# haotiansun14/rl-rep

Measured on NVIDIA B200. Metric: agent updates/sec, higher is better.
Workload: dtype tf32

## Files before the change

### rlrep_b200/csrc/gemm_chain.cu

```cuda
#include <algorithm>
#include <cmath>
#include <cstdlib>
#include <cstring>

#include "common.cuh"
#include "gemm_chain.cuh"
#include "ptx.cuh"

namespace rlrep {

namespace {

constexpr int kThreads = 320;
constexpr int kEpiWarps = 8;
constexpr int kStages = 6;
constexpr int kCW = 16;
constexpr int kTwPitch = kCW + 4;
constexpr int kMaxBn = 128;
constexpr int kBM = 128, kBK = 32;
constexpr int kABytes = kBM * kBK * 4;
constexpr int kStageBytes = kABytes + kMaxBn * kBK * 4;
constexpr int kTbufFloats = kEpiWarps * 32 * kTwPitch;
constexpr int kSub = 4, kCtrStride = 32;
constexpr int kDbgItems = 16, kDbgEvents = 10;
constexpr int kSmemBytes = kStages * kStageBytes + 1024 + 256 + kTbufFloats * 4;
static_assert(kSmemBytes <= 227 * 1024, "chain kernel shared memory");

__device__ __forceinline__ void red_release_add(unsigned* p, unsigned v) {
  asm volatile("red.release.gpu.global.add.u32 [%0], %1;" ::"l"(p), "r"(v) : "memory");
}
__device__ __forceinline__ unsigned atom_add_acq_rel(unsigned* p, unsigned v) {
  unsigned old;
  asm volatile("atom.acq_rel.gpu.global.add.u32 %0, [%1], %2;" : "=r"(old) : "l"(p), "r"(v) : "memory");
  return old;
}
__device__ __forceinline__ void fence_proxy_async_global() { asm volatile("fence.proxy.async.global;" ::: "memory"); }
__device__ __forceinline__ void fence_tensormap_acquire(const CUtensorMap* m) {
  asm volatile("fence.proxy.tensormap::generic.acquire.gpu [%0], 128;" ::"l"(reinterpret_cast<uint64_t>(m)) : "memory");
}
__device__ __forceinline__ unsigned ld_relaxed(const unsigned* p) {
  unsigned v;
  asm volatile("ld.relaxed.gpu.global.u32 %0, [%1];" : "=r"(v) : "l"(p) : "memory");
  return v;
}
__device__ __forceinline__ void wait_counter(const unsigned* done, int dep, int dep_tiles) {
  const unsigned* p = done + (size_t)dep * kSub * kCtrStride;
  unsigned target[kSub];
#pragma unroll
  for (int sub = 0; sub < kSub; ++sub) target[sub] = (unsigned)((dep_tiles - sub + kSub - 1) / kSub);
  long long t0 = 0;
  while (true) {
    unsigned v[kSub];
#pragma unroll
    for (int sub = 0; sub < kSub; ++sub) v[sub] = ld_relaxed(p + sub * kCtrStride);
    bool ok = true;
#pragma unroll
    for (int sub = 0; sub < kSub; ++sub) ok = ok && v[sub] >= target[sub];
    if (ok) return;
    __nanosleep(20);
    if (t0 == 0) t0 = clock64();
    if (clock64() - t0 > 4000000000LL) {
      printf("rlrep: chain dependency wait timed out (block %d, gemm %d, tiles %d, counters %u %u %u %u)\n", blockIdx.x, dep,
             dep_tiles, v[0], v[1], v[2], v[3]);
      __trap();
    }
  }
}
__device__ __forceinline__ void fence_acquire_gpu() { asm volatile("fence.acq_rel.gpu;" ::: "memory"); }

__device__ __forceinline__ void epilogue_bar() { asm volatile("bar.sync 1, 256;" ::: "memory"); }

__device__ __forceinline__ float elu_fast(float x) {
  const float n = fminf(x, 0.f);
  float p = 1.f / 5040.f;
  p = fmaf(p, n, 1.f / 720.f);
  p = fmaf(p, n, 1.f / 120.f);
  p = fmaf(p, n, 1.f / 24.f);
  p = fmaf(p, n, 1.f / 6.f);
  p = fmaf(p, n, 0.5f);
  p = fmaf(p, n, 1.f);
// ... 62 lines not shown
      if constexpr (ACT != ACT_NONE) {
#pragma unroll
        for (int e = 0; e < 4; ++e) v[e] = ACT == ACT_ELU ? elu_fast(v[e]) : apply_act(v[e], ACT < 0 ? epi.act : ACT);
      }
      if constexpr (DACT != DACT_NONE) {
        const int dact = DACT < 0 ? epi.dact : DACT;
        if (dact != DACT_NONE) {
          const float4 x = o.aux[r4];
          v[0] *= apply_dact(x.x, dact); v[1] *= apply_dact(x.y, dact); v[2] *= apply_dact(x.z, dact); v[3] *= apply_dact(x.w, dact);
        }
      }
      float4* cp = reinterpret_cast<float4*>(C + (size_t)om * ldc + on);
      if (epi.accumulate) {
        const float4 c0 = __ldcg(cp);
        v[0] += c0.x; v[1] += c0.y; v[2] += c0.z; v[3] += c0.w;
      }
      *cp = make_float4(v[0], v[1], v[2], v[3]);
    }
  }
}

__global__ void __launch_bounds__(kThreads, 1)
gemm_chain_kernel(const ChainGemmDesc* __restrict__ gemms, const ChainTask* __restrict__ tasks,
                  const int* __restrict__ task_begin, unsigned* __restrict__ done, unsigned* __restrict__ exit_ctr,
                  int n_gemms, unsigned long long* __restrict__ dbg) {
  auto stamp = [&](int item, int ev) {
    if (dbg != nullptr && item < kDbgItems) {
      unsigned long long t;
      asm volatile("mov.u64 %0, %%globaltimer;" : "=l"(t)::"memory");
      dbg[((size_t)blockIdx.x * kDbgItems + item) * kDbgEvents + ev] = t;
    }
  };
  if (threadIdx.x == 0) stamp(kDbgItems - 1, 2);
  extern __shared__ uint8_t smem_raw[];
  uint8_t* smem = reinterpret_cast<uint8_t*>((reinterpret_cast<uintptr_t>(smem_raw) + 1023) & ~uintptr_t(1023));
  uint64_t* full_bar = reinterpret_cast<uint64_t*>(smem + kStages * kStageBytes);
  uint64_t* empty_bar = full_bar + 8;
  uint64_t* acc_full = empty_bar + 8;
  uint64_t* acc_empty = acc_full + 2;
  uint32_t* tmem_slot = reinterpret_cast<uint32_t*>(acc_empty + 2);
  volatile unsigned* arrival = reinterpret_cast<volatile unsigned*>(tmem_slot + 1);
  float* tbuf = reinterpret_cast<float*>(smem + kStages * kStageBytes + 256);

  const int warp = threadIdx.x >> 5, lane = threadIdx.x & 31;
  const int t_begin = task_begin[blockIdx.x], t_end = task_begin[blockIdx.x + 1];

  if (threadIdx.x == 0) {
    for (int s = 0; s < kStages; ++s) {
      ptx::mbar_init(&full_bar[s], 1);
      ptx::mbar_init(&empty_bar[s], 1);
    }
    for (int a = 0; a < 2; ++a) {
      ptx::mbar_init(&acc_full[a], 1);
      ptx::mbar_init(&acc_empty[a], kEpiWarps);
    }
    ptx::fence_mbar_init();
  }
  if (warp == 1) {
    ptx::tmem_alloc(tmem_slot, 2 * kMaxBn);
    ptx::tmem_relinquish();
  }
  ptx::tc_fence_before_sync();
  __syncthreads();
  ptx::tc_fence_after_sync();
  const uint32_t tmem_base = *tmem_slot;

  if (warp == 0) {
    if (lane == 0) {
      int it = 0, last_gemm = -1;
      for (int t = t_begin; t < t_end; ++t) {
        const ChainTask tk = tasks[t];
        const ChainGemmDesc* g = gemms + tk.gemm;
        const int n_deps = g->n_deps;
        const int bn = g->bn, a_mn = g->a_mn, b_mn = g->b_mn;
        const int m0 = (tk.tile % g->tiles_m) * kBM, n0 = (tk.tile / g->tiles_m) * bn;
        const int kb0 = tk.split * g->kb_per_split, kb1 = min(g->nkb, kb0 + g->kb_per_split);
        int dep_id[kChainMaxDeps], dep_tiles[kChainMaxDeps];
#pragma unroll
        for (int d = 0; d < kChainMaxDeps; ++d) {
          dep_id[d] = d < n_deps ? g->dep[d] : 0;
          dep_tiles[d] = d < n_deps ? (int)g->dep_target[d] : 0;
        }
        if (tk.gemm != last_gemm) {
          fence_tensormap_acquire(&g->tmA);
          fence_tensormap_acquire(&g->tmB);
          last_gemm = tk.gemm;
        }
        stamp(t - t_begin, 0);
        if (dbg != nullptr && t - t_begin < kDbgItems)
          dbg[((size_t)blockIdx.x * kDbgItems + (t - t_begin)) * kDbgEvents + 8] =
              (unsigned long long)tk.gemm | ((unsigned long long)tk.tile << 16) | ((unsigned long long)tk.split << 40);
#pragma unroll
        for (int d = 0; d < kChainMaxDeps; ++d)
          if (d < n_deps) wait_counter(done, dep_id[d], dep_tiles[d]);
        if (n_deps > 0) {
          fence_acquire_gpu();
          fence_proxy_async_global();
        }
        stamp(t - t_begin, 1);
        const uint32_t tx = kABytes + bn * kBK * 4;
        for (int kb = kb0; kb < kb1; ++kb, ++it) {
          const int s = it % kStages;
          ptx::mbar_wait(&empty_bar[s], ((it / kStages) & 1) ^ 1);
          ptx::mbar_arrive_expect_tx(&full_bar[s], tx);
          uint8_t* a_dst = smem + s * kStageBytes;
          uint8_t* b_dst = a_dst + kABytes;
          const int k0 = kb * kBK;
          if (!a_mn) ptx::tma_load_2d(a_dst, &g->tmA, &full_bar[s], k0, m0);
          else ptx::tma_load_3d(a_dst, &g->tmA, &full_bar[s], 0, k0, m0 / 32);
          if (!b_mn) ptx::tma_load_2d(b_dst, &g->tmB, &full_bar[s], k0, n0);
          else ptx::tma_load_3d(b_dst, &g->tmB, &full_bar[s], 0, k0, n0 / 32);
        }
        stamp(t - t_begin, 2);
      }
    }
  } else if (warp == 1) {
    if (ptx::elect_one()) {
      int it = 0, tc = 0;
      for (int t = t_begin; t < t_end; ++t, ++tc) {
        const ChainTask tk = tasks[t];
        const ChainGemmDesc* g = gemms + tk.gemm;
        const int bn = g->bn, a_mn = g->a_mn, b_mn = g->b_mn;
        const int kb0 = tk.split * g->kb_per_split, kb1 = min(g->nkb, kb0 + g->kb_per_split);
        const uint32_t idesc = ptx::make_idesc_tf32(kBM, bn, a_mn != 0, b_mn != 0);
        const int acc = tc & 1;
        ptx::mbar_wait(&acc_empty[acc], ((tc >> 1) & 1) ^ 1);
        ptx::tc_fence_after_sync();
        const uint32_t d_tmem = tmem_base + acc * kMaxBn;
        for (int kb = kb0; kb < kb1; ++kb, ++it) {
          const int s = it % kStages;
          ptx::mbar_wait(&full_bar[s], (it / kStages) & 1);
          if (kb == kb0) stamp(t - t_begin, 3);
          ptx::tc_fence_after_sync();
          const uint32_t a_addr = ptx::smem_u32(smem + s * kStageBytes);
          const uint32_t b_addr = a_addr + kABytes;
#pragma unroll
          for (int k = 0; k < kBK / 8; ++k) {
            const uint64_t adesc = a_mn ? ptx::make_smem_desc(a_addr + k * 1024, 4096, 512, 1)
                                        : ptx::make_smem_desc(a_addr + k * 32, 16, 1024, 2);
            const uint64_t bdesc = b_mn ? ptx::make_smem_desc(b_addr + k * 1024, 4096, 512, 1)
                                        : ptx::make_smem_desc(b_addr + k * 32, 16, 1024, 2);
            ptx::mma_tf32_ss(d_tmem, adesc, bdesc, idesc, (kb > kb0 || k > 0) ? 1u : 0u);
          }
          ptx::mma_commit(&empty_bar[s]);
        }
        ptx::mma_commit(&acc_full[acc]);
        stamp(t - t_begin, 4);
      }
    }
  } else {
    const int q = warp & 3, half = (warp - 2) >> 2;
    float* tw = tbuf + (warp - 2) * (32 * kTwPitch);
    int tc = 0;
    for (int t = t_begin; t < t_end; ++t, ++tc) {
      const ChainTask tk = tasks[t];
      const ChainGemmDesc* g = gemms + tk.gemm;
      const Epilogue epi = g->epi;
      const int bn = g->bn, M = g->M, N = g->N, ldc = g->ldc, split_k = g->split_k;
      float* __restrict__ C = g->C;
      float* __restrict__ ws = g->ws;
      unsigned* __restrict__ tile_ctr = g->tile_ctr;
      const int m0 = (tk.tile % g->tiles_m) * kBM, n0 = (tk.tile / g->tiles_m) * bn;
      const int chunks = bn / kCW;
      const int acc = tc & 1;
      const uint32_t t_acc = tmem_base + (static_cast<uint32_t>(32 * q) << 16) + acc * kMaxBn;
      const int row = 32 * q + lane;
      ptx::mbar_wait(&acc_full[acc], (tc >> 1) & 1);
      if (threadIdx.x == 64) stamp(t - t_begin, 5);
      ptx::tc_fence_after_sync();

      bool final = true;
      const size_t part_floats = (size_t)kBM * bn;
      float* ws_tile = split_k > 1 ? ws + (size_t)tk.tile * split_k * part_floats : nullptr;
      const bool dist = split_k > 1 && g->dist != 0;
      int c_first = half, c_step = 2;
      if (split_k > 1) {
        float* part = ws_tile + (size_t)tk.split * part_floats;
#pragma unroll 1
        for (int c = half; c < chunks; c += 2) {
          if (dist && c % split_k == tk.split) continue;
          uint32_t v[kCW];
          ptx::tmem_ld_32x32b_x16(t_acc + c * kCW, v);
          ptx::tmem_ld_wait();
#pragma unroll
          for (int j = 0; j < kCW / 4; ++j)
            __stcg(reinterpret_cast<float4*>(part + ((size_t)(c * (kCW / 4) + j) * kBM + row) * 4),
                   make_float4(__uint_as_float(v[4 * j]), __uint_as_float(v[4 * j + 1]), __uint_as_float(v[4 * j + 2]),
                               __uint_as_float(v[4 * j + 3])));
        }
        epilogue_bar();
        if (threadIdx.x == 64) {
          unsigned* ctr = tile_ctr + tk.tile;
          const unsigned old = atom_add_acq_rel(ctr, 1u);
          if (dist) {
            if (old + 1 < (unsigned)split_k) {
              unsigned long long t0 = 0;
              unsigned spins = 0;
              while (ld_relaxed(ctr) < (unsigned)split_k) {
                __nanosleep(20);
                if ((++spins & 0xfff) == 0) {
                  unsigned long long now;
                  asm volatile("mov.u64 %0, %%globaltimer;" : "=l"(now));
                  if (t0 == 0) t0 = now;
                  else if (now - t0 > 2000000000ull) __trap();
                }
              }
              fence_acquire_gpu();
            }
          } else if (old == (unsigned)(split_k - 1)) {
            *ctr = 0;
          }
          *arrival = old;
          stamp(t - t_begin, 6);
        }
        epilogue_bar();
        final = dist || *arrival == (unsigned)(split_k - 1);
        if (dist) {
          c_first = tk.split + split_k * half;
          c_step = 2 * split_k;
        }
      }
      if (final) {
        const bool use_aux = epi.dact != DACT_NONE;
        const bool vec_ok = (ldc & 3) == 0 && aligned16(C) && (N & 3) == 0 &&
                            (!use_aux || ((epi.ld_aux & 3) == 0 && aligned16(epi.aux))) &&
                            (!epi.pre_out || ((epi.ld_pre & 3) == 0 && aligned16(epi.pre_out))) &&
                            (!epi.bias || aligned16(epi.bias)) && (!epi.r1_v || aligned16(epi.r1_v));
#pragma unroll 1
        for (int c = c_first; c < chunks; c += c_step) {
          const int gn0 = n0 + c * kCW;
          const bool fast = vec_ok && gn0 + kCW <= N;
          ChunkOperands ops;
          if (fast) chunk_prefetch(ops, epi, M, m0 + 32 * q, gn0, lane);
          float a[kCW];
          if (split_k == 1) {
            uint32_t v[kCW];
            ptx::tmem_ld_32x32b_x16(t_acc + c * kCW, v);
            ptx::tmem_ld_wait();
#pragma unroll
            for (int e = 0; e < kCW; ++e) a[e] = __uint_as_float(v[e]);
          } else {
            const float* base = ws_tile + ((size_t)(c * (kCW / 4)) * kBM + row) * 4;
            float4 nxt[kCW / 4];
            const int s_first = tk.split == 0 ? 1 : 0;
#pragma unroll
            for (int j = 0; j < kCW / 4; ++j)
              nxt[j] = __ldcg(reinterpret_cast<const float4*>(base + (size_t)s_first * part_floats + (size_t)j * kBM * 4));
#pragma unroll 1
            for (int s = 0; s < split_k; ++s) {
              if (s == tk.split) {
                uint32_t v[kCW];
                ptx::tmem_ld_32x32b_x16(t_acc + c * kCW, v);
                ptx::tmem_ld_wait();
                if (s == 0) {
#pragma unroll
                  for (int e = 0; e < kCW; ++e) a[e] = __uint_as_float(v[e]);
                } else {
#pragma unroll
                  for (int e = 0; e < kCW; ++e) a[e] += __uint_as_float(v[e]);
                }
                continue;
              }
              float4 cur[kCW / 4];
// ... 21 lines not shown
          __syncwarp();
          if (fast) {
#define RLREP_CSTORE(A, D) chain_store_rows<A, D>(epi, ops, tw, C, ldc, M, m0 + 32 * q, gn0, lane)
            RLREP_EPILOGUE_SWITCH(epi, RLREP_CSTORE);
#undef RLREP_CSTORE
          } else if (gn0 < N) {
            const int piece = lane & 3, rsub = lane >> 2;
#pragma unroll 1
            for (int r4 = 0; r4 < 4; ++r4) {
              const int r = r4 * 8 + rsub, om = m0 + 32 * q + r;
              if (om >= M) continue;
#pragma unroll 1
              for (int e = 0; e < 4; ++e) {
                const int on = gn0 + 4 * piece + e;
                if (on < N) {
                  float* cp = C + (size_t)om * ldc + on;
                  *cp = chain_epilogue_scalar(epi, tw[r * kTwPitch + 4 * piece + e], om, on, cp);
                }
              }
            }
          }
          __syncwarp();
        }
        if (threadIdx.x == 64) stamp(t - t_begin, 9);
        epilogue_bar();
        if (threadIdx.x == 64) {
          fence_proxy_async_global();
          const int pub = dist ? tk.tile * split_k + tk.split : tk.tile;
          red_release_add(done + ((size_t)tk.gemm * kSub + (pub % kSub)) * kCtrStride, 1u);
          stamp(t - t_begin, 7);
          if (dist) {
            unsigned* ctr = tile_ctr + tk.tile;
            if (atomicAdd(ctr, 1u) == (unsigned)(2 * split_k - 1)) *ctr = 0;
          }
        }
      }
      ptx::tc_fence_before_sync();
      __syncwarp();
      if (lane == 0) ptx::mbar_arrive(&acc_empty[acc]);
    }
  }
  ptx::tc_fence_before_sync();
  __syncthreads();
  if (warp == 1) ptx::tmem_dealloc(tmem_base, 2 * kMaxBn);
  if (threadIdx.x == 0) {
    const unsigned old = atom_add_acq_rel(exit_ctr, 1u);
    if (old == gridDim.x - 1) {
      for (int i = 0; i < n_gemms * kSub; ++i) done[(size_t)i * kCtrStride] = 0;
      *exit_ctr = 0;
      __threadfence();
    }
    stamp(kDbgItems - 1, 3);
  }
}

struct Range {
  uintptr_t lo = 0, hi = 0;
  bool overlaps(const Range& o) const { return lo < o.hi && o.lo < hi && lo != hi && o.lo != o.hi; }
};
Range range_of(const float* p, long long rows, long long ld, long long cols) {
  Range r;
  if (p == nullptr || rows <= 0 || cols <= 0) return r;
  r.lo = reinterpret_cast<uintptr_t>(p);
  r.hi = r.lo + (size_t)((rows - 1) * ld + cols) * sizeof(float);
  return r;
}
struct Footprint {
  std::vector<Range> reads, writes;
};
Footprint footprint(const GemmArgs& a) {
  Footprint f;
  f.reads.push_back(a.a_mn ? range_of(a.A, a.K, a.lda, a.M) : range_of(a.A, a.M, a.lda, a.K));
  f.reads.push_back(a.b_mn ? range_of(a.B, a.K, a.ldb, a.N) : range_of(a.B, a.N, a.ldb, a.K));
  f.reads.push_back(range_of(a.epi.bias, 1, 0, a.N));
// ... 5 lines not shown
  f.writes.push_back(range_of(a.epi.pre_out, a.M, a.epi.ld_pre, a.N));
  return f;
}
bool conflicts(const Footprint& earlier, const Footprint& later) {
  for (const Range& w : earlier.writes) {
    for (const Range& r : later.reads)
      if (w.overlaps(r)) return true;
    for (const Range& r : later.writes)
      if (w.overlaps(r)) return true;
  }
  for (const Range& w : later.writes)
    for (const Range& r : earlier.reads)
      if (w.overlaps(r)) return true;
  return false;
}

unsigned long long* g_chain_dbg = nullptr;

int env_int(const char* name, int dflt) {
  const char* e = std::getenv(name);
  return e ? std::atoi(e) : dflt;
}

bool dist_possible(int bn, int split) { return split > 1 && (bn / kCW) % split == 0; }
double plan_cost(int tiles, int nkb, int bn, int split, int share, bool dist) {
  const int kb_per = ceil_div(nkb, split);
  const double kb_bytes = kABytes + bn * kBK * 4;
  const double waves = std::ceil((double)tiles * split / share);
  const double stream = waves * kb_per * kb_bytes / 150e3;
  const double chip = (double)tiles * split * kb_per * kb_bytes / 12e6;
  if (dist) {
    return 1.5 + std::max(stream, chip) + waves * (0.25 * ceil_div(bn, 64) + 1.0 + 1.0 * ceil_div(bn / split, 64)) +
           0.1 * (split - 1);
  }
  double t = 1.5 + std::max(stream, chip) + waves * 1.0 * ceil_div(bn, 64);
  if (split > 1) t += 1.5 + 0.3 * (split - 1) * ceil_div(bn, 64);
  return t;
}

}

void set_chain_debug_buffer(unsigned long long* dev) { g_chain_dbg = dev; }

bool chain_eligible(const GemmArgs& a) {
  return tc_eligible(a) && a.conv_w == 0 && a.M >= 32 && a.N >= 32 && a.K >= 8;
}

GemmChain::~GemmChain() {
  if (dev_) cudaFree(dev_);
}

bool GemmChain::matches(const std::vector<GemmArgs>& seq) const {
  if (seq.size() != seq_.size()) return false;
  for (size_t i = 0; i < seq.size(); ++i) {
// ... 9 lines not shown
}

void GemmChain::build(const std::vector<GemmArgs>& seq, int force_bn, int force_split) {
  RLREP_CHECK(dev_ == nullptr, "chain already built");
  RLREP_CHECK(!seq.empty(), "empty chain");
  const int n = (int)seq.size();
  for (const GemmArgs& a : seq) RLREP_CHECK(chain_eligible(a), "GEMM cannot be a member of a chain");
  seq_ = seq;
  int n_sm = kNumSMs;
  {
    int dev = 0;
    RLREP_CUDA(cudaGetDevice(&dev));
    RLREP_CUDA(cudaDeviceGetAttribute(&n_sm, cudaDevAttrMultiProcessorCount, dev));
  }
  static bool attr_set = false;
  if (!attr_set) {
    RLREP_CUDA(cudaFuncSetAttribute(gemm_chain_kernel, cudaFuncAttributeMaxDynamicSharedMemorySize, kSmemBytes));
    attr_set = true;
  }
  int per_sm = 0;
  RLREP_CUDA(cudaOccupancyMaxActiveBlocksPerMultiprocessor(&per_sm, gemm_chain_kernel, kThreads, kSmemBytes));
  RLREP_CHECK(per_sm >= 1, "chain kernel does not fit on an SM");
  const int n_cta = n_sm;

  std::vector<Footprint> fp(n);
  for (int i = 0; i < n; ++i) fp[i] = footprint(seq[i]);
  std::vector<std::vector<int>> deps(n);
  std::vector<std::vector<char>> reach(n, std::vector<char>(n, 0));
  std::vector<int> level(n, 0);
  for (int j = 0; j < n; ++j) {
    std::vector<int> direct;
    for (int i = 0; i < j; ++i)
      if (conflicts(fp[i], fp[j])) direct.push_back(i);
    for (int i : direct) {
      reach[j][i] = 1;
      for (int k = 0; k < n; ++k)
        if (reach[i][k]) reach[j][k] = 1;
    }
    for (int i : direct) {
      bool implied = false;
      for (int k : direct)
        if (k != i && reach[k][i]) implied = true;
      if (!implied) deps[j].push_back(i);
      level[j] = std::max(level[j], level[i] + 1);
    }
    RLREP_CHECK((int)deps[j].size() <= kChainMaxDeps, "a chain GEMM has too many direct dependencies");
  }
  levels_ = 1 + *std::max_element(level.begin(), level.end());

  std::vector<int> bn(n), split(n), share(n), first_cta(n), dist(n, 0);
  const int dist_mode = env_int("RLREP_CHAIN_DIST", 1);
  auto work_of = [&](int i) {
    return (double)ceil_div(seq[i].M, kBM) * ceil_div(seq[i].N, kMaxBn) * ceil_div(seq[i].K, kBK);
  };
  auto items_of = [&](int i) { return ceil_div(seq[i].M, kBM) * ceil_div(seq[i].N, bn[i]) * (dist[i] ? split[i] : 1); };
  for (int L = 0; L < levels_; ++L) {
    std::vector<int> members;
    for (int i = 0; i < n; ++i)
      if (level[i] == L) members.push_back(i);
    double total = 0.0;
    for (int i : members) total += work_of(i);
    int cursor = 0, seen = 0;
    for (int i : members) {
      const GemmArgs& a = seq[i];
      const int nkb = ceil_div(a.K, kBK);
      ++seen;
      int sh = std::max(4, (int)std::floor(n_cta * work_of(i) / total));
      if (seen == (int)members.size()) sh = std::max(sh, n_cta - cursor);
      sh = std::min(sh, n_cta);
      first_cta[i] = cursor % n_cta;
      cursor += sh;
      share[i] = sh;
      double best = 1e300;
      for (int cbn : {32, 64, 128}) {
        if (force_bn && cbn != force_bn) continue;
        if (!force_bn && cbn > 32 && cbn / 2 >= a.N) continue;
        const int tiles = ceil_div(a.M, kBM) * ceil_div(a.N, cbn);
        for (int s : {1, 2, 4, 8, 16}) {
          if (force_split && s != force_split) continue;
          if (s > 1 && (s - 1) * ceil_div(nkb, s) >= nkb) continue;
          for (int d = 0; d < 2; ++d) {
            if (d == 1 && (dist_mode == 0 || !dist_possible(cbn, s) || tiles * s > sh)) continue;
            if (d == 0 && dist_mode == 2 && dist_possible(cbn, s) && tiles * s <= sh) continue;
            const double c = plan_cost(tiles, nkb, cbn, s, sh, d == 1);
            if (c < best - 1e-9) {
              best = c;
              bn[i] = cbn;
              split[i] = s;
              dist[i] = d;
            }
          }
        }
      }
      if (best > 1e299) {
        bn[i] = force_bn ? force_bn : 32;
        split[i] = 1;
        dist[i] = 0;
      }
    }
  }

  std::vector<std::vector<ChainTask>> per_cta(n_cta);
  std::vector<int> order(n);
  for (int i = 0; i < n; ++i) order[i] = i;
  std::stable_sort(order.begin(), order.end(), [&](int x, int y) { return level[x] < level[y]; });
  size_t ws_floats = 0, ctr_count = 0;
  std::vector<size_t> ws_off(n, 0), ctr_off(n, 0);
  std::vector<ChainGemmDesc> descs(n);
  bytes_ = flops_ = 0.0;
  for (int i : order) {
    const GemmArgs& a = seq[i];
    const int tiles_m = ceil_div(a.M, kBM), tiles_n = ceil_div(a.N, bn[i]);
    const int tiles = tiles_m * tiles_n;
    int item = 0;
    for (int t = 0; t < tiles; ++t)
      for (int s = 0; s < split[i]; ++s, ++item)
        per_cta[(first_cta[i] + item % share[i]) % n_cta].push_back(ChainTask{i, t, s, 0});
    ChainGemmDesc& d = descs[i];
    std::memset(&d, 0, sizeof(d));
    d.tmA = make_operand_map(a.A, a.a_mn, a.M, a.K, a.lda, kBM);
    d.tmB = make_operand_map(a.B, a.b_mn, a.N, a.K, a.ldb, bn[i]);
    d.epi = a.epi;
    d.C = a.C;
    d.ldc = a.ldc; d.M = a.M; d.N = a.N; d.K = a.K;
    d.bn = bn[i]; d.a_mn = a.a_mn; d.b_mn = a.b_mn; d.nkb = ceil_div(a.K, kBK);
    d.split_k = split[i]; d.kb_per_split = ceil_div(d.nkb, split[i]);
    d.dist = dist[i];
    d.tiles_m = tiles_m; d.tiles_n = tiles_n;
    d.n_deps = (int)deps[i].size();
    for (int k = 0; k < d.n_deps; ++k) {
      const int j = deps[i][k];
      d.dep[k] = j;
      d.dep_target[k] = (unsigned)items_of(j);
    }
    ctr_off[i] = ctr_count;
    ctr_count += (size_t)tiles;
    if (split[i] > 1) {
      ws_off[i] = ws_floats;
      ws_floats += (size_t)tiles * split[i] * kBM * bn[i];
    }
    bytes_ += 4.0 * ((double)a.M * a.K + (double)a.N * a.K + (double)a.M * a.N);
    flops_ += 2.0 * a.M * a.N * a.K;
  }
  std::vector<ChainTask> tasks;
  std::vector<int> begin(n_cta + 1, 0);
  for (int c = 0; c < n_cta; ++c) {
    begin[c] = (int)tasks.size();
    tasks.insert(tasks.end(), per_cta[c].begin(), per_cta[c].end());
  }
  begin[n_cta] = (int)tasks.size();
  grid_ = n_cta;

  auto up = [](size_t x) { return (x + 255) & ~size_t(255); };
  const size_t o_desc = 0;
  const size_t o_tasks = up(o_desc + sizeof(ChainGemmDesc) * n);
  const size_t o_begin = up(o_tasks + sizeof(ChainTask) * tasks.size());
  const size_t o_done = up(o_begin + sizeof(int) * begin.size());
  const size_t o_exit = up(o_done + sizeof(unsigned) * n * kSub * kCtrStride);
  const size_t o_ctr = up(o_exit + sizeof(unsigned));
  const size_t o_ws = up(o_ctr + sizeof(unsigned) * ctr_count);
  const size_t total_bytes = o_ws + sizeof(float) * ws_floats + 256;
  RLREP_CUDA(cudaMalloc(&dev_, total_bytes));
  RLREP_CUDA(cudaMemset(dev_, 0, o_ws));
  char* base = static_cast<char*>(dev_);
  d_gemms_ = reinterpret_cast<ChainGemmDesc*>(base + o_desc);
  d_tasks_ = reinterpret_cast<ChainTask*>(base + o_tasks);
  d_task_begin_ = reinterpret_cast<int*>(base + o_begin);
  d_done_ = reinterpret_cast<unsigned*>(base + o_done);
  d_exit_ = reinterpret_cast<unsigned*>(base + o_exit);
  for (int i = 0; i < n; ++i) {
    descs[i].tile_ctr = reinterpret_cast<unsigned*>(base + o_ctr) + ctr_off[i];
    descs[i].ws = split[i] > 1 ? reinterpret_cast<float*>(base + o_ws) + ws_off[i] : nullptr;
  }
  RLREP_CUDA(cudaMemcpy(d_gemms_, descs.data(), sizeof(ChainGemmDesc) * n, cudaMemcpyHostToDevice));
  RLREP_CUDA(cudaMemcpy(d_tasks_, tasks.data(), sizeof(ChainTask) * tasks.size(), cudaMemcpyHostToDevice));
  RLREP_CUDA(cudaMemcpy(d_task_begin_, begin.data(), sizeof(int) * begin.size(), cudaMemcpyHostToDevice));
  RLREP_CUDA(cudaDeviceSynchronize());
  if (env_int("RLREP_CHAIN_VERBOSE", 0)) {
    std::fprintf(stderr, "rlrep chain: %d GEMMs, %d levels, %zu items, ws %.1f MB\n", n, levels_, tasks.size(),
                 ws_floats * 4 / 1e6);
    for (int i = 0; i < n; ++i)
      std::fprintf(stderr, "  [%d] L%d M=%d N=%d K=%d a_mn=%d b_mn=%d bn=%d split=%d%s share=%d deps=%d\n", i, level[i],
                   seq[i].M, seq[i].N, seq[i].K, (int)seq[i].a_mn, (int)seq[i].b_mn, bn[i], split[i],
                   dist[i] ? " (distributed)" : "", share[i], (int)deps[i].size());
  }
}

void GemmChain::launch(cudaStream_t stream) {
  RLREP_CHECK(dev_ != nullptr, "chain not built");
  cudaLaunchConfig_t cfg = {};
  cfg.gridDim = dim3(grid_);
  cfg.blockDim = dim3(kThreads);
  cfg.dynamicSmemBytes = kSmemBytes;
  cfg.stream = stream;
  cudaLaunchAttribute attr[1];
  attr[0].id = cudaLaunchAttributeCooperative;
  attr[0].val.cooperative = 1;
  cfg.attrs = attr;
  cfg.numAttrs = 1;
  RLREP_CUDA(cudaLaunchKernelEx(&cfg, gemm_chain_kernel, (const ChainGemmDesc*)d_gemms_, (const ChainTask*)d_tasks_,
                                (const int*)d_task_begin_, d_done_, d_exit_, (int)seq_.size(), g_chain_dbg));
  RLREP_LAUNCHED_W("gemm_chain", stream, bytes_, flops_);
}

}
```

### rlrep_b200/csrc/gemm_chain.cuh

```cuda
#pragma once
#include <vector>

#include "gemm.cuh"

namespace rlrep {

constexpr int kChainMaxDeps = 6;

struct alignas(128) ChainGemmDesc {
  CUtensorMap tmA;
  CUtensorMap tmB;
  Epilogue epi;
  int dist;
  float* C;
  float* ws;
  unsigned* tile_ctr;
  int ldc, M, N, K;
  int bn, a_mn, b_mn, nkb;
  int split_k, kb_per_split, tiles_m, tiles_n;
  int n_deps;
  int dep[kChainMaxDeps];
  unsigned dep_target[kChainMaxDeps];
};

struct ChainTask {
  int gemm, tile, split, pad;
};

class GemmChain {
 public:
  GemmChain() = default;
  GemmChain(const GemmChain&) = delete;
  GemmChain& operator=(const GemmChain&) = delete;
  ~GemmChain();
  bool matches(const std::vector<GemmArgs>& seq) const;
  void build(const std::vector<GemmArgs>& seq, int force_bn = 0, int force_split = 0);
  void launch(cudaStream_t stream);
  int size() const { return (int)seq_.size(); }
  int levels() const { return levels_; }

 private:
  std::vector<GemmArgs> seq_;
  void* dev_ = nullptr;
  ChainGemmDesc* d_gemms_ = nullptr;
  ChainTask* d_tasks_ = nullptr;
  int* d_task_begin_ = nullptr;
  unsigned* d_done_ = nullptr;
  unsigned* d_exit_ = nullptr;
  int grid_ = 0, levels_ = 0;
  double bytes_ = 0.0, flops_ = 0.0;
};

void set_chain_debug_buffer(unsigned long long* dev);

bool chain_eligible(const GemmArgs& a);

}
```

### rlrep_b200/csrc/ptx.cuh

```cuda
#pragma once
#include <cstdint>
#include <cuda.h>
#include <cuda_runtime.h>

namespace rlrep {
namespace ptx {

__device__ __forceinline__ uint32_t smem_u32(const void* p) {
  return static_cast<uint32_t>(__cvta_generic_to_shared(p));
}

__device__ __forceinline__ bool elect_one() {
  uint32_t pred = 0;
  asm volatile(
      "{\n"
      ".reg .b32 rx;\n"
      ".reg .pred px;\n"
      "elect.sync rx|px, 0xffffffff;\n"
      "selp.u32 %0, 1, 0, px;\n"
      "}\n"
      : "=r"(pred));
  return pred != 0;
}

__device__ __forceinline__ void mbar_init(uint64_t* bar, uint32_t count) {
  asm volatile("mbarrier.init.shared::cta.b64 [%0], %1;" ::"r"(smem_u32(bar)), "r"(count) : "memory");
}
__device__ __forceinline__ void fence_mbar_init() {
  asm volatile("fence.mbarrier_init.release.cluster;" ::: "memory");
}
__device__ __forceinline__ void fence_proxy_async_smem() {
  asm volatile("fence.proxy.async.shared::cta;" ::: "memory");
}
__device__ __forceinline__ void mbar_arrive_expect_tx(uint64_t* bar, uint32_t bytes) {
  asm volatile("mbarrier.arrive.expect_tx.shared::cta.b64 _, [%0], %1;" ::"r"(smem_u32(bar)), "r"(bytes)
               : "memory");
}
__device__ __forceinline__ void mbar_arrive(uint64_t* bar) {
  asm volatile("mbarrier.arrive.shared::cta.b64 _, [%0];" ::"r"(smem_u32(bar)) : "memory");
}
__device__ __forceinline__ bool mbar_try_wait(uint64_t* bar, uint32_t parity) {
  uint32_t ok;
  asm volatile(
      "{\n"
      ".reg .pred p;\n"
      "mbarrier.try_wait.parity.shared::cta.b64 p, [%1], %2;\n"
      "selp.u32 %0, 1, 0, p;\n"
      "}\n"
      : "=r"(ok)
      : "r"(smem_u32(bar)), "r"(parity)
      : "memory");
  return ok != 0;
}
__device__ __forceinline__ void mbar_wait(uint64_t* bar, uint32_t parity) {
  if (mbar_try_wait(bar, parity)) return;
  const long long t0 = clock64();
  while (!mbar_try_wait(bar, parity)) {
    if (clock64() - t0 > 4000000000LL) {
      printf("rlrep: mbarrier wait timed out (block %d,%d,%d thread %d)\n", blockIdx.x, blockIdx.y,
             blockIdx.z, threadIdx.x);
      __trap();
    }
  }
}

__device__ __forceinline__ void prefetch_tensormap(const CUtensorMap* m) {
  asm volatile("prefetch.tensormap [%0];" ::"l"(reinterpret_cast<uint64_t>(m)) : "memory");
}
__device__ __forceinline__ void tma_load_2d(void* smem_dst, const CUtensorMap* m, uint64_t* bar, int c_inner,
                                            int c_outer) {
  asm volatile(
      "cp.async.bulk.tensor.2d.shared::cluster.global.mbarrier::complete_tx::bytes [%0], [%1, {%3, %4}], [%2];"
      ::"r"(smem_u32(smem_dst)),
      "l"(reinterpret_cast<uint64_t>(m)), "r"(smem_u32(bar)), "r"(c_inner), "r"(c_outer)
      : "memory");
}
__device__ __forceinline__ void tma_load_3d(void* smem_dst, const CUtensorMap* m, uint64_t* bar, int c0, int c1, int c2) {
  asm volatile(
      "cp.async.bulk.tensor.3d.shared::cluster.global.mbarrier::complete_tx::bytes [%0], [%1, {%3, %4, %5}], [%2];"
      ::"r"(smem_u32(smem_dst)),
// ... 77 lines not shown
__device__ __forceinline__ void cluster_arrive() {
  asm volatile("barrier.cluster.arrive.release.aligned;" ::: "memory");
}
__device__ __forceinline__ void cluster_arrive_relaxed() {
  asm volatile("barrier.cluster.arrive.relaxed.aligned;" ::: "memory");
}
__device__ __forceinline__ void cluster_wait() {
  asm volatile("barrier.cluster.wait.acquire.aligned;" ::: "memory");
}
__device__ __forceinline__ uint32_t cluster_ctarank() {
  uint32_t r;
  asm volatile("mov.u32 %0, %%cluster_ctarank;" : "=r"(r));
  return r;
}
__device__ __forceinline__ float4 ld_shared_f4(uint32_t addr) {
  float4 v;
  asm volatile("ld.shared.v4.f32 {%0, %1, %2, %3}, [%4];" : "=f"(v.x), "=f"(v.y), "=f"(v.z), "=f"(v.w) : "r"(addr) : "memory");
  return v;
}
__device__ __forceinline__ void st_dsmem_f4(uint32_t addr, uint32_t cta_rank, float4 v) {
  uint32_t remote;
  asm volatile("mapa.shared::cluster.u32 %0, %1, %2;" : "=r"(remote) : "r"(addr), "r"(cta_rank));
  asm volatile("st.shared::cluster.v4.f32 [%0], {%1, %2, %3, %4};" ::"r"(remote), "f"(v.x), "f"(v.y), "f"(v.z), "f"(v.w)
               : "memory");
}
__device__ __forceinline__ float4 ld_dsmem_f4(uint32_t addr, uint32_t cta_rank) {
  uint32_t remote;
  asm volatile("mapa.shared::cluster.u32 %0, %1, %2;" : "=r"(remote) : "r"(addr), "r"(cta_rank));
  float4 v;
  asm volatile("ld.shared::cluster.v4.f32 {%0, %1, %2, %3}, [%4];"
               : "=f"(v.x), "=f"(v.y), "=f"(v.z), "=f"(v.w)
               : "r"(remote)
               : "memory");
  return v;
}

__device__ __forceinline__ uint64_t make_smem_desc(uint32_t smem_addr, uint32_t lbo_bytes, uint32_t sbo_bytes,
                                                   uint32_t layout) {
  uint64_t d = 0;
  d |= static_cast<uint64_t>((smem_addr >> 4) & 0x3FFF);
  d |= static_cast<uint64_t>((lbo_bytes >> 4) & 0x3FFF) << 16;
  d |= static_cast<uint64_t>((sbo_bytes >> 4) & 0x3FFF) << 32;
  d |= static_cast<uint64_t>(1) << 46;
  d |= static_cast<uint64_t>(layout) << 61;
  return d;
}
// ... 9 lines not shown
```

Before: 1280.

## Add CTA-pair DSMEM split-K reduction, operand prefetch before dependency wait, launch-epoch counters

Adds a split-2 reduction mode in which paired CTAs of a 2-CTA cluster exchange half of their TMEM accumulators through st.async into the peer's shared memory, replacing the global workspace round trip. The producer can also issue TMA loads for an operand no earlier GEMM writes before waiting on dependencies. The end-of-kernel reset of the done counters by the last CTA is replaced by per-CTA launch counts that offset the wait targets. Pipeline stages drop from 6 to 5 to free shared memory for the receive buffer, which may reduce latency hiding.

```diff
diff --git a/rlrep_b200/csrc/gemm_chain.cu b/rlrep_b200/csrc/gemm_chain.cu
--- a/rlrep_b200/csrc/gemm_chain.cu
+++ b/rlrep_b200/csrc/gemm_chain.cu
@@ -13,7 +13,7 @@
 
 constexpr int kThreads = 320;
 constexpr int kEpiWarps = 8;
-constexpr int kStages = 6;
+constexpr int kStages = 5;
 constexpr int kCW = 16;
 constexpr int kTwPitch = kCW + 4;
 constexpr int kMaxBn = 128;
@@ -21,9 +21,10 @@
 constexpr int kABytes = kBM * kBK * 4;
 constexpr int kStageBytes = kABytes + kMaxBn * kBK * 4;
 constexpr int kTbufFloats = kEpiWarps * 32 * kTwPitch;
+constexpr int kRecvFloats = kBM * kMaxBn / 2;
 constexpr int kSub = 4, kCtrStride = 32;
 constexpr int kDbgItems = 16, kDbgEvents = 10;
-constexpr int kSmemBytes = kStages * kStageBytes + 1024 + 256 + kTbufFloats * 4;
+constexpr int kSmemBytes = kStages * kStageBytes + 1024 + 256 + kTbufFloats * 4 + kRecvFloats * 4;
 static_assert(kSmemBytes <= 227 * 1024, "chain kernel shared memory");
 
 __device__ __forceinline__ void red_release_add(unsigned* p, unsigned v) {
@@ -43,11 +44,14 @@
   asm volatile("ld.relaxed.gpu.global.u32 %0, [%1];" : "=r"(v) : "l"(p) : "memory");
   return v;
 }
-__device__ __forceinline__ void wait_counter(const unsigned* done, int dep, int dep_tiles) {
+__device__ __forceinline__ void wait_counter(const unsigned* done, int dep, int dep_tiles, unsigned launch) {
   const unsigned* p = done + (size_t)dep * kSub * kCtrStride;
-  unsigned target[kSub];
-#pragma unroll
-  for (int sub = 0; sub < kSub; ++sub) target[sub] = (unsigned)((dep_tiles - sub + kSub - 1) / kSub);
+  unsigned target[kSub], base[kSub];
+#pragma unroll
+  for (int sub = 0; sub < kSub; ++sub) {
+    target[sub] = (unsigned)((dep_tiles - sub + kSub - 1) / kSub);
+    base[sub] = launch * target[sub];
+  }
   long long t0 = 0;
   while (true) {
     unsigned v[kSub];
@@ -55,7 +59,7 @@
     for (int sub = 0; sub < kSub; ++sub) v[sub] = ld_relaxed(p + sub * kCtrStride);
     bool ok = true;
 #pragma unroll
-    for (int sub = 0; sub < kSub; ++sub) ok = ok && v[sub] >= target[sub];
+    for (int sub = 0; sub < kSub; ++sub) ok = ok && v[sub] - base[sub] >= target[sub];
     if (ok) return;
     __nanosleep(20);
     if (t0 == 0) t0 = clock64();
@@ -164,8 +168,8 @@
 
 __global__ void __launch_bounds__(kThreads, 1)
 gemm_chain_kernel(const ChainGemmDesc* __restrict__ gemms, const ChainTask* __restrict__ tasks,
-                  const int* __restrict__ task_begin, unsigned* __restrict__ done, unsigned* __restrict__ exit_ctr,
-                  int n_gemms, unsigned long long* __restrict__ dbg) {
+                  const int* __restrict__ task_begin, unsigned* __restrict__ done, unsigned* __restrict__ launches,
+                  int paired, unsigned long long* __restrict__ dbg) {
   auto stamp = [&](int item, int ev) {
     if (dbg != nullptr && item < kDbgItems) {
       unsigned long long t;
@@ -180,9 +184,12 @@
   uint64_t* empty_bar = full_bar + 8;
   uint64_t* acc_full = empty_bar + 8;
   uint64_t* acc_empty = acc_full + 2;
-  uint32_t* tmem_slot = reinterpret_cast<uint32_t*>(acc_empty + 2);
+  uint64_t* recv_full = acc_empty + 2;
+  uint64_t* peer_free = recv_full + 1;
+  uint32_t* tmem_slot = reinterpret_cast<uint32_t*>(peer_free + 1);
   volatile unsigned* arrival = reinterpret_cast<volatile unsigned*>(tmem_slot + 1);
   float* tbuf = reinterpret_cast<float*>(smem + kStages * kStageBytes + 256);
+  float* recv = tbuf + kTbufFloats;
 
   const int warp = threadIdx.x >> 5, lane = threadIdx.x & 31;
   const int t_begin = task_begin[blockIdx.x], t_end = task_begin[blockIdx.x + 1];
@@ -196,6 +203,8 @@
       ptx::mbar_init(&acc_full[a], 1);
       ptx::mbar_init(&acc_empty[a], kEpiWarps);
     }
+    ptx::mbar_init(recv_full, 1);
+    ptx::mbar_init(peer_free, kEpiWarps);
     ptx::fence_mbar_init();
   }
   if (warp == 1) {
@@ -203,13 +212,15 @@
     ptx::tmem_relinquish();
   }
   ptx::tc_fence_before_sync();
-  __syncthreads();
+  if (paired) ptx::cluster_sync();
+  else __syncthreads();
   ptx::tc_fence_after_sync();
   const uint32_t tmem_base = *tmem_slot;
 
   if (warp == 0) {
     if (lane == 0) {
       int it = 0, last_gemm = -1;
+      const unsigned launch = launches[blockIdx.x];
       for (int t = t_begin; t < t_end; ++t) {
         const ChainTask tk = tasks[t];
         const ChainGemmDesc* g = gemms + tk.gemm;
@@ -232,26 +243,43 @@
         if (dbg != nullptr && t - t_begin < kDbgItems)
           dbg[((size_t)blockIdx.x * kDbgItems + (t - t_begin)) * kDbgEvents + 8] =
               (unsigned long long)tk.gemm | ((unsigned long long)tk.tile << 16) | ((unsigned long long)tk.split << 40);
+        const uint32_t tx = kABytes + bn * kBK * 4;
+        auto load_a = [&](int kb, int s) {
+          uint8_t* dst = smem + s * kStageBytes;
+          if (!a_mn) ptx::tma_load_2d(dst, &g->tmA, &full_bar[s], kb * kBK, m0);
+          else ptx::tma_load_3d(dst, &g->tmA, &full_bar[s], 0, kb * kBK, m0 / 32);
+        };
+        auto load_b = [&](int kb, int s) {
+          uint8_t* dst = smem + s * kStageBytes + kABytes;
+          if (!b_mn) ptx::tma_load_2d(dst, &g->tmB, &full_bar[s], kb * kBK, n0);
+          else ptx::tma_load_3d(dst, &g->tmB, &full_bar[s], 0, kb * kBK, n0 / 32);
+        };
+        const int pre = n_deps > 0 ? g->prefetch : 0;
+        const int n_pre = pre ? min(kb1 - kb0, kStages) : 0;
+        for (int i = 0; i < n_pre; ++i) {
+          const int s = (it + i) % kStages;
+          ptx::mbar_wait(&empty_bar[s], (((it + i) / kStages) & 1) ^ 1);
+          ptx::mbar_arrive_expect_tx(&full_bar[s], tx);
+          if (pre == 1) load_a(kb0 + i, s);
+          else load_b(kb0 + i, s);
+        }
 #pragma unroll
         for (int d = 0; d < kChainMaxDeps; ++d)
-          if (d < n_deps) wait_counter(done, dep_id[d], dep_tiles[d]);
+          if (d < n_deps) wait_counter(done, dep_id[d], dep_tiles[d], launch);
         if (n_deps > 0) {
           fence_acquire_gpu();
           fence_proxy_async_global();
         }
         stamp(t - t_begin, 1);
-        const uint32_t tx = kABytes + bn * kBK * 4;
         for (int kb = kb0; kb < kb1; ++kb, ++it) {
           const int s = it % kStages;
-          ptx::mbar_wait(&empty_bar[s], ((it / kStages) & 1) ^ 1);
-          ptx::mbar_arrive_expect_tx(&full_bar[s], tx);
-          uint8_t* a_dst = smem + s * kStageBytes;
-          uint8_t* b_dst = a_dst + kABytes;
-          const int k0 = kb * kBK;
-          if (!a_mn) ptx::tma_load_2d(a_dst, &g->tmA, &full_bar[s], k0, m0);
-          else ptx::tma_load_3d(a_dst, &g->tmA, &full_bar[s], 0, k0, m0 / 32);
-          if (!b_mn) ptx::tma_load_2d(b_dst, &g->tmB, &full_bar[s], k0, n0);
-          else ptx::tma_load_3d(b_dst, &g->tmB, &full_bar[s], 0, k0, n0 / 32);
+          const bool claimed = kb - kb0 < n_pre;
+          if (!claimed) {
+            ptx::mbar_wait(&empty_bar[s], ((it / kStages) & 1) ^ 1);
+            ptx::mbar_arrive_expect_tx(&full_bar[s], tx);
+          }
+          if (!claimed || pre != 1) load_a(kb, s);
+          if (!claimed || pre != 2) load_b(kb, s);
         }
         stamp(t - t_begin, 2);
       }
@@ -293,7 +321,7 @@
   } else {
     const int q = warp & 3, half = (warp - 2) >> 2;
     float* tw = tbuf + (warp - 2) * (32 * kTwPitch);
-    int tc = 0;
+    int tc = 0, pk = 0;
     for (int t = t_begin; t < t_end; ++t, ++tc) {
       const ChainTask tk = tasks[t];
       const ChainGemmDesc* g = gemms + tk.gemm;
@@ -313,10 +341,29 @@
 
       bool final = true;
       const size_t part_floats = (size_t)kBM * bn;
-      float* ws_tile = split_k > 1 ? ws + (size_t)tk.tile * split_k * part_floats : nullptr;
       const bool dist = split_k > 1 && g->dist != 0;
-      int c_first = half, c_step = 2;
-      if (split_k > 1) {
+      const bool pair = split_k > 1 && g->dist == 2;
+      const uint32_t peer = tk.split ^ 1;
+      float* ws_tile = split_k > 1 && !pair ? ws + (size_t)tk.tile * split_k * part_floats : nullptr;
+      const int c_first = dist ? tk.split + split_k * half : half, c_step = dist ? 2 * split_k : 2;
+      if (pair) {
+        if (threadIdx.x == 64) ptx::mbar_arrive_expect_tx(recv_full, (uint32_t)(kBM * (bn / 2) * 4));
+        ptx::mbar_wait(peer_free, (pk & 1) ^ 1, true);
+        const uint32_t dst = ptx::smem_u32(recv) + (uint32_t)row * 16;
+#pragma unroll 1
+        for (int j = half; j < chunks / 2; j += 2) {
+          uint32_t v[kCW];
+          ptx::tmem_ld_32x32b_x16(t_acc + (2 * j + peer) * kCW, v);
+          ptx::tmem_ld_wait();
+#pragma unroll
+          for (int jj = 0; jj < kCW / 4; ++jj)
+            ptx::st_async_dsmem_f4(dst + (uint32_t)(j * (kCW / 4) + jj) * kBM * 16, recv_full, peer,
+                                   make_float4(__uint_as_float(v[4 * jj]), __uint_as_float(v[4 * jj + 1]),
+                                               __uint_as_float(v[4 * jj + 2]), __uint_as_float(v[4 * jj + 3])));
+        }
+        ptx::mbar_wait(recv_full, pk & 1, true);
+        if (threadIdx.x == 64) stamp(t - t_begin, 6);
+      } else if (split_k > 1) {
         float* part = ws_tile + (size_t)tk.split * part_floats;
 #pragma unroll 1
         for (int c = half; c < chunks; c += 2) {
@@ -357,10 +404,6 @@
         }
         epilogue_bar();
         final = dist || *arrival == (unsigned)(split_k - 1);
-        if (dist) {
-          c_first = tk.split + split_k * half;
-          c_step = 2 * split_k;
-        }
       }
       if (final) {
         const bool use_aux = epi.dact != DACT_NONE;
@@ -381,6 +424,23 @@
             ptx::tmem_ld_wait();
 #pragma unroll
             for (int e = 0; e < kCW; ++e) a[e] = __uint_as_float(v[e]);
+          } else if (pair) {
+            const float* rp = recv + ((size_t)(c / 2 * (kCW / 4)) * kBM + row) * 4;
+            float4 p[kCW / 4];
+#pragma unroll
+            for (int j = 0; j < kCW / 4; ++j) p[j] = *reinterpret_cast<const float4*>(rp + (size_t)j * kBM * 4);
+            uint32_t v[kCW];
+            ptx::tmem_ld_32x32b_x16(t_acc + c * kCW, v);
+            ptx::tmem_ld_wait();
+#pragma unroll
+            for (int j = 0; j < kCW / 4; ++j) {
+              const float o[4] = {p[j].x, p[j].y, p[j].z, p[j].w};
+#pragma unroll
+              for (int e = 0; e < 4; ++e) {
+                const float mine = __uint_as_float(v[4 * j + e]);
+                a[4 * j + e] = tk.split == 0 ? mine + o[e] : o[e] + mine;
+              }
+            }
           } else {
             const float* base = ws_tile + ((size_t)(c * (kCW / 4)) * kBM + row) * 4;
             float4 nxt[kCW / 4];
@@ -448,6 +508,10 @@
           }
           __syncwarp();
         }
+        if (pair) {
+          if (lane == 0) ptx::mbar_arrive_remote(peer_free, peer);
+          ++pk;
+        }
         if (threadIdx.x == 64) stamp(t - t_begin, 9);
         epilogue_bar();
         if (threadIdx.x == 64) {
@@ -455,7 +519,7 @@
           const int pub = dist ? tk.tile * split_k + tk.split : tk.tile;
           red_release_add(done + ((size_t)tk.gemm * kSub + (pub % kSub)) * kCtrStride, 1u);
           stamp(t - t_begin, 7);
-          if (dist) {
+          if (dist && !pair) {
             unsigned* ctr = tile_ctr + tk.tile;
             if (atomicAdd(ctr, 1u) == (unsigned)(2 * split_k - 1)) *ctr = 0;
           }
@@ -467,15 +531,11 @@
     }
   }
   ptx::tc_fence_before_sync();
-  __syncthreads();
+  if (paired) ptx::cluster_sync();
+  else __syncthreads();
   if (warp == 1) ptx::tmem_dealloc(tmem_base, 2 * kMaxBn);
   if (threadIdx.x == 0) {
-    const unsigned old = atom_add_acq_rel(exit_ctr, 1u);
-    if (old == gridDim.x - 1) {
-      for (int i = 0; i < n_gemms * kSub; ++i) done[(size_t)i * kCtrStride] = 0;
-      *exit_ctr = 0;
-      __threadfence();
-    }
+    launches[blockIdx.x] += 1u;
     stamp(kDbgItems - 1, 3);
   }
 }
@@ -527,14 +587,18 @@
   return e ? std::atoi(e) : dflt;
 }
 
+enum { kRedLast = 0, kRedDist = 1, kRedPair = 2 };
 bool dist_possible(int bn, int split) { return split > 1 && (bn / kCW) % split == 0; }
-double plan_cost(int tiles, int nkb, int bn, int split, int share, bool dist) {
+double plan_cost(int tiles, int nkb, int bn, int split, int share, int red) {
   const int kb_per = ceil_div(nkb, split);
   const double kb_bytes = kABytes + bn * kBK * 4;
   const double waves = std::ceil((double)tiles * split / share);
   const double stream = waves * kb_per * kb_bytes / 150e3;
   const double chip = (double)tiles * split * kb_per * kb_bytes / 12e6;
-  if (dist) {
+  if (red == kRedPair) {
+    return 1.5 + std::max(stream, chip) + waves * (0.5 + 1.0 * ceil_div(bn / 2, 64));
+  }
+  if (red == kRedDist) {
     return 1.5 + std::max(stream, chip) + waves * (0.25 * ceil_div(bn, 64) + 1.0 + 1.0 * ceil_div(bn / split, 64)) +
            0.1 * (split - 1);
   }
@@ -590,6 +654,24 @@
   RLREP_CUDA(cudaOccupancyMaxActiveBlocksPerMultiprocessor(&per_sm, gemm_chain_kernel, kThreads, kSmemBytes));
   RLREP_CHECK(per_sm >= 1, "chain kernel does not fit on an SM");
   const int n_cta = n_sm;
+  const int dist_mode = env_int("RLREP_CHAIN_DIST", 1);
+  bool pair_ok = n_cta % 2 == 0 && (dist_mode == 1 || dist_mode == 3);
+  if (pair_ok) {
+    cudaLaunchConfig_t cfg = {};
+    cfg.gridDim = dim3(n_cta);
+    cfg.blockDim = dim3(kThreads);
+    cfg.dynamicSmemBytes = kSmemBytes;
+    cudaLaunchAttribute attr[1];
+    attr[0].id = cudaLaunchAttributeClusterDimension;
+    attr[0].val.clusterDim.x = 2;
+    attr[0].val.clusterDim.y = 1;
+    attr[0].val.clusterDim.z = 1;
+    cfg.attrs = attr;
+    cfg.numAttrs = 1;
+    int clusters = 0;
+    RLREP_CUDA(cudaOccupancyMaxActiveClusters(&clusters, gemm_chain_kernel, &cfg));
+    pair_ok = clusters >= n_cta / 2;
+  }
 
   std::vector<Footprint> fp(n);
   for (int i = 0; i < n; ++i) fp[i] = footprint(seq[i]);
@@ -617,7 +699,6 @@
   levels_ = 1 + *std::max_element(level.begin(), level.end());
 
   std::vector<int> bn(n), split(n), share(n), first_cta(n), dist(n, 0);
-  const int dist_mode = env_int("RLREP_CHAIN_DIST", 1);
   auto work_of = [&](int i) {
     return (double)ceil_div(seq[i].M, kBM) * ceil_div(seq[i].N, kMaxBn) * ceil_div(seq[i].K, kBK);
   };
@@ -647,10 +728,14 @@
         for (int s : {1, 2, 4, 8, 16}) {
           if (force_split && s != force_split) continue;
           if (s > 1 && (s - 1) * ceil_div(nkb, s) >= nkb) continue;
-          for (int d = 0; d < 2; ++d) {
-            if (d == 1 && (dist_mode == 0 || !dist_possible(cbn, s) || tiles * s > sh)) continue;
-            if (d == 0 && dist_mode == 2 && dist_possible(cbn, s) && tiles * s <= sh) continue;
-            const double c = plan_cost(tiles, nkb, cbn, s, sh, d == 1);
+          const bool dist_ok = dist_mode != 0 && dist_possible(cbn, s) && tiles * s <= sh;
+          const bool pair_here = pair_ok && s == 2 && dist_ok && tiles * 2 <= sh - (first_cta[i] & 1);
+          for (int d = kRedLast; d <= kRedPair; ++d) {
+            if (d == kRedDist && !dist_ok) continue;
+            if (d == kRedPair && !pair_here) continue;
+            if (d != kRedDist && dist_mode == 2 && dist_ok) continue;
+            if (d != kRedPair && dist_mode == 3 && pair_here) continue;
+            const double c = plan_cost(tiles, nkb, cbn, s, sh, d);
             if (c < best - 1e-9) {
               best = c;
               bn[i] = cbn;
@@ -681,9 +766,15 @@
     const int tiles_m = ceil_div(a.M, kBM), tiles_n = ceil_div(a.N, bn[i]);
     const int tiles = tiles_m * tiles_n;
     int item = 0;
-    for (int t = 0; t < tiles; ++t)
-      for (int s = 0; s < split[i]; ++s, ++item)
-        per_cta[(first_cta[i] + item % share[i]) % n_cta].push_back(ChainTask{i, t, s, 0});
+    if (dist[i] == kRedPair) {
+      const int base = (first_cta[i] + 1) & ~1;
+      for (int t = 0; t < tiles; ++t)
+        for (int s = 0; s < 2; ++s) per_cta[(base + 2 * t + s) % n_cta].push_back(ChainTask{i, t, s, 0});
+    } else {
+      for (int t = 0; t < tiles; ++t)
+        for (int s = 0; s < split[i]; ++s, ++item)
+          per_cta[(first_cta[i] + item % share[i]) % n_cta].push_back(ChainTask{i, t, s, 0});
+    }
     ChainGemmDesc& d = descs[i];
     std::memset(&d, 0, sizeof(d));
     d.tmA = make_operand_map(a.A, a.a_mn, a.M, a.K, a.lda, kBM);
@@ -694,6 +785,13 @@
     d.bn = bn[i]; d.a_mn = a.a_mn; d.b_mn = a.b_mn; d.nkb = ceil_div(a.K, kBK);
     d.split_k = split[i]; d.kb_per_split = ceil_div(d.nkb, split[i]);
     d.dist = dist[i];
+    bool a_free = true, b_free = true;
+    for (int j = 0; j < i; ++j)
+      for (const Range& w : fp[j].writes) {
+        a_free = a_free && !w.overlaps(fp[i].reads[0]);
+        b_free = b_free && !w.overlaps(fp[i].reads[1]);
+      }
+    d.prefetch = b_free ? 2 : a_free ? 1 : 0;
     d.tiles_m = tiles_m; d.tiles_n = tiles_n;
     d.n_deps = (int)deps[i].size();
     for (int k = 0; k < d.n_deps; ++k) {
@@ -703,7 +801,7 @@
     }
     ctr_off[i] = ctr_count;
     ctr_count += (size_t)tiles;
-    if (split[i] > 1) {
+    if (split[i] > 1 && dist[i] != kRedPair) {
       ws_off[i] = ws_floats;
       ws_floats += (size_t)tiles * split[i] * kBM * bn[i];
     }
@@ -718,14 +816,28 @@
   }
   begin[n_cta] = (int)tasks.size();
   grid_ = n_cta;
+  paired_ = false;
+  for (int p = 0; 2 * p + 1 < n_cta; ++p) {
+    std::vector<ChainTask> half[2];
+    for (int s = 0; s < 2; ++s)
+      for (const ChainTask& tk : per_cta[2 * p + s])
+        if (descs[tk.gemm].dist == kRedPair) half[s].push_back(tk);
+    RLREP_CHECK(half[0].size() == half[1].size(), "pair items are not mirrored in a CTA pair");
+    for (size_t k = 0; k < half[0].size(); ++k)
+      RLREP_CHECK(half[0][k].gemm == half[1][k].gemm && half[0][k].tile == half[1][k].tile && half[0][k].split == 0 &&
+                      half[1][k].split == 1,
+                  "pair items are not mirrored in a CTA pair");
+    paired_ = paired_ || !half[0].empty();
+  }
+  RLREP_CHECK(!paired_ || pair_ok, "pair reductions planned without a CTA-pair launch");
 
   auto up = [](size_t x) { return (x + 255) & ~size_t(255); };
   const size_t o_desc = 0;
   const size_t o_tasks = up(o_desc + sizeof(ChainGemmDesc) * n);
   const size_t o_begin = up(o_tasks + sizeof(ChainTask) * tasks.size());
   const size_t o_done = up(o_begin + sizeof(int) * begin.size());
-  const size_t o_exit = up(o_done + sizeof(unsigned) * n * kSub * kCtrStride);
-  const size_t o_ctr = up(o_exit + sizeof(unsigned));
+  const size_t o_launches = up(o_done + sizeof(unsigned) * n * kSub * kCtrStride);
+  const size_t o_ctr = up(o_launches + sizeof(unsigned) * n_cta);
   const size_t o_ws = up(o_ctr + sizeof(unsigned) * ctr_count);
   const size_t total_bytes = o_ws + sizeof(float) * ws_floats + 256;
   RLREP_CUDA(cudaMalloc(&dev_, total_bytes));
@@ -735,10 +847,10 @@
   d_tasks_ = reinterpret_cast<ChainTask*>(base + o_tasks);
   d_task_begin_ = reinterpret_cast<int*>(base + o_begin);
   d_done_ = reinterpret_cast<unsigned*>(base + o_done);
-  d_exit_ = reinterpret_cast<unsigned*>(base + o_exit);
+  d_launches_ = reinterpret_cast<unsigned*>(base + o_launches);
   for (int i = 0; i < n; ++i) {
     descs[i].tile_ctr = reinterpret_cast<unsigned*>(base + o_ctr) + ctr_off[i];
-    descs[i].ws = split[i] > 1 ? reinterpret_cast<float*>(base + o_ws) + ws_off[i] : nullptr;
+    descs[i].ws = split[i] > 1 && dist[i] != kRedPair ? reinterpret_cast<float*>(base + o_ws) + ws_off[i] : nullptr;
   }
   RLREP_CUDA(cudaMemcpy(d_gemms_, descs.data(), sizeof(ChainGemmDesc) * n, cudaMemcpyHostToDevice));
   RLREP_CUDA(cudaMemcpy(d_tasks_, tasks.data(), sizeof(ChainTask) * tasks.size(), cudaMemcpyHostToDevice));
@@ -750,7 +862,7 @@
     for (int i = 0; i < n; ++i)
       std::fprintf(stderr, "  [%d] L%d M=%d N=%d K=%d a_mn=%d b_mn=%d bn=%d split=%d%s share=%d deps=%d\n", i, level[i],
                    seq[i].M, seq[i].N, seq[i].K, (int)seq[i].a_mn, (int)seq[i].b_mn, bn[i], split[i],
-                   dist[i] ? " (distributed)" : "", share[i], (int)deps[i].size());
+                   dist[i] == kRedPair ? " (pair)" : dist[i] ? " (distributed)" : "", share[i], (int)deps[i].size());
   }
 }
 
@@ -761,13 +873,18 @@
   cfg.blockDim = dim3(kThreads);
   cfg.dynamicSmemBytes = kSmemBytes;
   cfg.stream = stream;
-  cudaLaunchAttribute attr[1];
+  cudaLaunchAttribute attr[2];
   attr[0].id = cudaLaunchAttributeCooperative;
   attr[0].val.cooperative = 1;
+  attr[1].id = cudaLaunchAttributeClusterDimension;
+  attr[1].val.clusterDim.x = 2;
+  attr[1].val.clusterDim.y = 1;
+  attr[1].val.clusterDim.z = 1;
   cfg.attrs = attr;
-  cfg.numAttrs = 1;
+  cfg.numAttrs = paired_ ? 2 : 1;
   RLREP_CUDA(cudaLaunchKernelEx(&cfg, gemm_chain_kernel, (const ChainGemmDesc*)d_gemms_, (const ChainTask*)d_tasks_,
-                                (const int*)d_task_begin_, d_done_, d_exit_, (int)seq_.size(), g_chain_dbg));
+                                (const int*)d_task_begin_, d_done_, d_launches_, (int)paired_,
+                                g_chain_dbg));
   RLREP_LAUNCHED_W("gemm_chain", stream, bytes_, flops_);
 }
 
diff --git a/rlrep_b200/csrc/gemm_chain.cuh b/rlrep_b200/csrc/gemm_chain.cuh
--- a/rlrep_b200/csrc/gemm_chain.cuh
+++ b/rlrep_b200/csrc/gemm_chain.cuh
@@ -12,6 +12,7 @@
   CUtensorMap tmB;
   Epilogue epi;
   int dist;
+  int prefetch;
   float* C;
   float* ws;
   unsigned* tile_ctr;
@@ -46,8 +47,9 @@
   ChainTask* d_tasks_ = nullptr;
   int* d_task_begin_ = nullptr;
   unsigned* d_done_ = nullptr;
-  unsigned* d_exit_ = nullptr;
+  unsigned* d_launches_ = nullptr;
   int grid_ = 0, levels_ = 0;
+  bool paired_ = false;
   double bytes_ = 0.0, flops_ = 0.0;
 };
 
diff --git a/rlrep_b200/csrc/ptx.cuh b/rlrep_b200/csrc/ptx.cuh
--- a/rlrep_b200/csrc/ptx.cuh
+++ b/rlrep_b200/csrc/ptx.cuh
@@ -39,23 +39,39 @@
 __device__ __forceinline__ void mbar_arrive(uint64_t* bar) {
   asm volatile("mbarrier.arrive.shared::cta.b64 _, [%0];" ::"r"(smem_u32(bar)) : "memory");
 }
-__device__ __forceinline__ bool mbar_try_wait(uint64_t* bar, uint32_t parity) {
+__device__ __forceinline__ void mbar_arrive_remote(uint64_t* bar, uint32_t cta_rank) {
+  uint32_t remote;
+  asm volatile("mapa.shared::cluster.u32 %0, %1, %2;" : "=r"(remote) : "r"(smem_u32(bar)), "r"(cta_rank));
+  asm volatile("mbarrier.arrive.release.cluster.shared::cluster.b64 _, [%0];" ::"r"(remote) : "memory");
+}
+__device__ __forceinline__ bool mbar_try_wait(uint64_t* bar, uint32_t parity, bool cluster = false) {
   uint32_t ok;
-  asm volatile(
-      "{\n"
-      ".reg .pred p;\n"
-      "mbarrier.try_wait.parity.shared::cta.b64 p, [%1], %2;\n"
-      "selp.u32 %0, 1, 0, p;\n"
-      "}\n"
-      : "=r"(ok)
-      : "r"(smem_u32(bar)), "r"(parity)
-      : "memory");
+  if (cluster)
+    asm volatile(
+        "{\n"
+        ".reg .pred p;\n"
+        "mbarrier.try_wait.parity.acquire.cluster.shared::cta.b64 p, [%1], %2;\n"
+        "selp.u32 %0, 1, 0, p;\n"
+        "}\n"
+        : "=r"(ok)
+        : "r"(smem_u32(bar)), "r"(parity)
+        : "memory");
+  else
+    asm volatile(
+        "{\n"
+        ".reg .pred p;\n"
+        "mbarrier.try_wait.parity.shared::cta.b64 p, [%1], %2;\n"
+        "selp.u32 %0, 1, 0, p;\n"
+        "}\n"
+        : "=r"(ok)
+        : "r"(smem_u32(bar)), "r"(parity)
+        : "memory");
   return ok != 0;
 }
-__device__ __forceinline__ void mbar_wait(uint64_t* bar, uint32_t parity) {
-  if (mbar_try_wait(bar, parity)) return;
+__device__ __forceinline__ void mbar_wait(uint64_t* bar, uint32_t parity, bool cluster = false) {
+  if (mbar_try_wait(bar, parity, cluster)) return;
   const long long t0 = clock64();
-  while (!mbar_try_wait(bar, parity)) {
+  while (!mbar_try_wait(bar, parity, cluster)) {
     if (clock64() - t0 > 4000000000LL) {
       printf("rlrep: mbarrier wait timed out (block %d,%d,%d thread %d)\n", blockIdx.x, blockIdx.y,
              blockIdx.z, threadIdx.x);
@@ -179,6 +195,14 @@
   uint32_t remote;
   asm volatile("mapa.shared::cluster.u32 %0, %1, %2;" : "=r"(remote) : "r"(addr), "r"(cta_rank));
   asm volatile("st.shared::cluster.v4.f32 [%0], {%1, %2, %3, %4};" ::"r"(remote), "f"(v.x), "f"(v.y), "f"(v.z), "f"(v.w)
+               : "memory");
+}
+__device__ __forceinline__ void st_async_dsmem_f4(uint32_t addr, uint64_t* bar, uint32_t cta_rank, float4 v) {
+  uint32_t raddr, rbar;
+  asm volatile("mapa.shared::cluster.u32 %0, %1, %2;" : "=r"(raddr) : "r"(addr), "r"(cta_rank));
+  asm volatile("mapa.shared::cluster.u32 %0, %1, %2;" : "=r"(rbar) : "r"(smem_u32(bar)), "r"(cta_rank));
+  asm volatile("st.async.shared::cluster.mbarrier::complete_tx::bytes.v4.f32 [%0], {%1, %2, %3, %4}, [%5];" ::"r"(raddr),
+               "f"(v.x), "f"(v.y), "f"(v.z), "f"(v.w), "r"(rbar)
                : "memory");
 }
 __device__ __forceinline__ float4 ld_dsmem_f4(uint32_t addr, uint32_t cta_rank) {
```

After: 1293, median of 6. No clear change (+1.0%).
